# Heartfirey/UCOD-DPL

Measured on AMD Instinct MI355X. Metric: training images/sec at 3x518x518, DINOv2-B (frozen backbone fwd + DBA/APM/discriminator train step), higher is better.
Workload: dtype f16; 1 GPU; BASELINE configs[1]: dinov2_vitb14 @518x518, batch 32/GPU, full APM+DBA+discriminator step, decoder path f32 (1x1 conv as a three-way bf16 split on the matrix pipe: f32-equivalent), backbone fp16 MFMA; global_batch=32, parallelism=dp1, backbone_last_layer=key-minimal (identical key output; 279.6 of 303.1 GFLOP/img), random_init_weights=True, residual_stream=fp16, ln_fold=True

## Files before the change

ucod_dpl_amd/csrc/dba.hip:

```cpp
#include "common.h"
#include "../../include/ucod_dpl.h"

namespace ucod {

constexpr int E = 64;
constexpr float NORM_EPS = 1e-12f;

__global__ __launch_bounds__(256) void colnorm_kernel(const float* __restrict__ d, int ld_c, int c0, const float* __restrict__ emb,
                                                      float* __restrict__ norm, int HW) {
  __shared__ float red[16];
  const int c = blockIdx.x, b = blockIdx.y;
  const float e = emb[c];
  const float* row = d + ((long)b * ld_c + c0 + c) * HW;
  float s = 0.f;
#pragma unroll 8
  for (int p = threadIdx.x; p < HW; p += 256) {
    const float u = row[p] * e;
    s = fmaf(u, u, s);
  }
  s = block_sum(s, red);
  if (threadIdx.x == 0) norm[b * 128 + c] = fmaxf(sqrtf(s), NORM_EPS);
}

__global__ __launch_bounds__(256) void heads_fwd_kernel(const float* __restrict__ d, int ld_c, int c0, const float* __restrict__ emb,
                                                        const float* __restrict__ norm, const float* __restrict__ head_w,
                                                        const float* __restrict__ head_b, float* __restrict__ fg,
                                                        float* __restrict__ bg, float* __restrict__ sdiag, int HW) {
  __shared__ float kf[128], hw[128];
  __shared__ float red[16];
  const int b = blockIdx.y, tid = threadIdx.x;
  if (tid < 128) {
    kf[tid] = emb[tid] / norm[b * 128 + tid];
    hw[tid] = head_w[tid];
  }
  __syncthreads();
  const int p = blockIdx.x * 256 + tid;
  float s2 = 0.f;
  if (p < HW) {
    const float* dp = d + ((long)b * ld_c + c0) * HW + p;
    float accf = head_b[0], accb = head_b[1], s = 0.f;
    for (int c0 = 0; c0 < E; c0 += 16) {
      float v1[16], v2[16];
#pragma unroll
      for (int j = 0; j < 16; ++j) {
        v1[j] = dp[(long)(c0 + j) * HW];
        v2[j] = dp[(long)(c0 + j + E) * HW];
      }
      __builtin_amdgcn_sched_barrier(0);
#pragma unroll
      for (int j = 0; j < 16; ++j) {
        const int c = c0 + j;
        const float d1 = v1[j], d2 = v2[j];
        const float f1 = d1 * kf[c], f2 = d2 * kf[c + E];
        accf = fmaf(hw[c], sigmoid_gate(f1 * d1) + d1, accf);
        accb = fmaf(hw[c + E], sigmoid_gate(f2 * d2) + d2, accb);
        s = fmaf(f1, f2, s);
      }
    }
    fg[(long)b * HW + p] = accf;
    if (bg) bg[(long)b * HW + p] = accb;
    s2 = s * s;
  }
  if (sdiag) {
    s2 = block_sum(s2, red);
    if (tid == 0) atomicAdd(&sdiag[b], s2);
  }
}

constexpr int GCH = 512;
constexpr int GK = 64;
constexpr int GLD = 129;
__global__ __launch_bounds__(256, 2) void gram_partial_kernel(const float* __restrict__ d, int ld_c, int c0,
                                                           const float* __restrict__ emb, const float* __restrict__ norm,
                                                           float* __restrict__ partial, int HW, int S) {
  __shared__ float Fs[2][GK * GLD];
  const int tid = threadIdx.x, lane = tid & 63, wave = tid >> 6;
  const int b = blockIdx.y, ps = blockIdx.x * GCH, pe = min(ps + GCH, HW);
  const float* dbase = d + ((long)b * ld_c + c0) * HW;
  const int sk = tid & 63, srow = tid >> 6;
  const int br = wave >> 1, rt = wave & 1;
  float kf[32];
#pragma unroll
  for (int i = 0; i < 32; ++i) kf[i] = emb[srow + 4 * i] / norm[b * 128 + srow + 4 * i];
  f32x16 acc[2];
#pragma unroll
  for (int i = 0; i < 16; ++i) { acc[0][i] = 0.f; acc[1][i] = 0.f; }

  float r[32];
  auto gload = [&](int k0) {
    const int k = k0 + sk;
    const float* src = dbase + (k < pe ? k : pe - 1);
    const float live = k < pe ? 1.f : 0.f;
#pragma unroll
    for (int i = 0; i < 32; ++i) r[i] = src[(long)(srow + 4 * i) * HW];
#pragma unroll
    for (int i = 0; i < 32; ++i) r[i] *= kf[i] * live;
  };
  auto lstore = [&](int buf) {
#pragma unroll
    for (int i = 0; i < 32; ++i) Fs[buf][sk * GLD + srow + 4 * i] = r[i];
  };
  const int nt = (pe - ps + GK - 1) / GK;
  gload(ps);
  lstore(0);
  for (int t = 0; t < nt; ++t) {
    __syncthreads();
    const bool more = t + 1 < nt;
    if (more) gload(ps + (t + 1) * GK);
    const float* fs = Fs[t & 1];
#pragma unroll 8
    for (int kk = 0; kk < GK; kk += 2) {
      const int k = kk + (lane >> 5);
      const float a = fs[k * GLD + br * 64 + rt * 32 + (lane & 31)];
      const float b0 = fs[k * GLD + br * 64 + (lane & 31)];
      const float b1 = fs[k * GLD + br * 64 + 32 + (lane & 31)];
      acc[0] = __builtin_amdgcn_mfma_f32_32x32x2f32(a, b0, acc[0], 0, 0, 0);
      acc[1] = __builtin_amdgcn_mfma_f32_32x32x2f32(a, b1, acc[1], 0, 0, 0);
    }
    if (more) lstore((t + 1) & 1);
  }
  float* out = partial + (((long)b * S + blockIdx.x) * 2 + br) * (E * E);
#pragma unroll
  for (int ct = 0; ct < 2; ++ct)
#pragma unroll
    for (int rg = 0; rg < 16; ++rg) {
      const int i = rt * 32 + (rg & 3) + 8 * (rg >> 2) + 4 * (lane >> 5);
      const int j = ct * 32 + (lane & 31);
      out[i * E + j] = acc[ct][rg];
    }
}

constexpr int FIN_Y = E * E / 256;
__global__ __launch_bounds__(256) void gram_finalize_kernel(const float* __restrict__ partial, float* __restrict__ gram,
                                                            float* __restrict__ trace, int S) {
  __shared__ float red[16];
  const int b = blockIdx.x, i = blockIdx.y * 256 + threadIdx.x;
  float g1 = 0.f, g2 = 0.f;
  for (int s = 0; s < S; ++s) {
    const float* p = partial + (((long)b * S + s) * 2) * (E * E);
    g1 += p[i];
    g2 += p[E * E + i];
  }
  gram[((long)b * 2 + 0) * (E * E) + i] = g1;
  gram[((long)b * 2 + 1) * (E * E) + i] = g2;
  const float tr = block_sum(g1 * g2, red);
  if (threadIdx.x == 0) trace[b * FIN_Y + blockIdx.y] = tr;
}

__global__ void orth_loss_kernel(const float* __restrict__ trace, const float* __restrict__ sdiag, float* __restrict__ loss, int B,
                                 double inv_z) {
  if (threadIdx.x == 0 && blockIdx.x == 0) {
    double t = 0.0;
    for (int b = 0; b < B; ++b) {
      double tb = 0.0;
      for (int y = 0; y < FIN_Y; ++y) tb += (double)trace[b * FIN_Y + y];
      t += tb - (double)sdiag[b];
    }
    loss[0] = (float)(t * inv_z);
  }
}

__global__ __launch_bounds__(256, 2) void dba_bwd_a_kernel(const float* __restrict__ d, int ld_c, int c0, const float* __restrict__ emb,
                                                           const float* __restrict__ norm, const float* __restrict__ head_w,
                                                           const float* __restrict__ gram, const float* __restrict__ gfg,
                                                           const float* __restrict__ gbg, float coef ,
                                                           float* __restrict__ gfeat, int HW) {
  __shared__ float G[2][E * E];
  __shared__ float kf[128], hw[128];
  const int b = blockIdx.y, tid = threadIdx.x, lane = tid & 63, wave = tid >> 6;
  const int l31 = lane & 31, h5 = lane >> 5;
  for (int i = tid; i < 2 * E * E; i += 256) (&G[0][0])[i] = gram[(long)b * 2 * E * E + i];
  if (tid < 128) {
    kf[tid] = emb[tid] / norm[b * 128 + tid];
    hw[tid] = head_w[tid];
  }
  __syncthreads();
  const int pbase = blockIdx.x * 256 + wave * 64;
  int px[2];
  bool ok[2];
#pragma unroll
  for (int ct = 0; ct < 2; ++ct) {
    const int p = pbase + ct * 32 + l31;
    ok[ct] = p < HW;
    px[ct] = ok[ct] ? p : HW - 1;
  }
  const float* dp = d + ((long)b * ld_c + c0) * HW;

  f32x16 a1[2][2], a2[2][2];
#pragma unroll
  for (int i = 0; i < 16; ++i) {
    a1[0][0][i] = a1[0][1][i] = a1[1][0][i] = a1[1][1][i] = 0.f;
    a2[0][0][i] = a2[0][1][i] = a2[1][0][i] = a2[1][1][i] = 0.f;
  }
  float spart[2] = {0.f, 0.f};
  for (int kk0 = 0; kk0 < E; kk0 += 16) {
    float r1[8][2], r2[8][2];
#pragma unroll
    for (int j = 0; j < 8; ++j) {
      const int k = kk0 + 2 * j + h5;
#pragma unroll
      for (int ct = 0; ct < 2; ++ct) {
        r1[j][ct] = dp[(long)k * HW + px[ct]];
        r2[j][ct] = dp[(long)(k + E) * HW + px[ct]];
      }
    }
    __builtin_amdgcn_sched_barrier(0);
#pragma unroll
    for (int j = 0; j < 8; ++j) {
      const int k = kk0 + 2 * j + h5;
      const float k1 = kf[k], k2 = kf[E + k];
      float f1[2], f2[2];
#pragma unroll
      for (int ct = 0; ct < 2; ++ct) {
        f1[ct] = r1[j][ct] * k1;
        f2[ct] = r2[j][ct] * k2;
        spart[ct] = fmaf(f1[ct], f2[ct], spart[ct]);
      }
#pragma unroll
      for (int rt = 0; rt < 2; ++rt) {
        const float g2 = G[1][k * E + rt * 32 + l31];
        const float g1 = G[0][k * E + rt * 32 + l31];
#pragma unroll
        for (int ct = 0; ct < 2; ++ct) {
          a1[rt][ct] = __builtin_amdgcn_mfma_f32_32x32x2f32(g2, f1[ct], a1[rt][ct], 0, 0, 0);
          a2[rt][ct] = __builtin_amdgcn_mfma_f32_32x32x2f32(g1, f2[ct], a2[rt][ct], 0, 0, 0);
        }
      }
    }
  }
  float* gp = gfeat + (long)b * 128 * HW;
#pragma unroll
  for (int ct = 0; ct < 2; ++ct) {
    const float s = spart[ct] + __shfl_xor(spart[ct], 32, 64);
    const long gi = (long)b * HW + px[ct];
    const float g1 = gfg[gi], g2 = gbg[gi];
#pragma unroll
    for (int rt = 0; rt < 2; ++rt)
#pragma unroll
      for (int r = 0; r < 16; ++r) {
        const int c = rt * 32 + (r & 3) + 8 * (r >> 2) + 4 * h5;
        const float d1 = dp[(long)c * HW + px[ct]], d2 = dp[(long)(c + E) * HW + px[ct]];
        const float f1 = d1 * kf[c], f2 = d2 * kf[c + E];
        const float s1 = sigmoid_gate(f1 * d1), s2 = sigmoid_gate(f2 * d2);
        if (ok[ct]) {
          gp[(long)c * HW + px[ct]] = coef * (a1[rt][ct][r] - s * f2) + g1 * hw[c] * s1 * (1.f - s1) * d1;
          gp[(long)(c + E) * HW + px[ct]] = coef * (a2[rt][ct][r] - s * f1) + g2 * hw[c + E] * s2 * (1.f - s2) * d2;
        }
      }
  }
}

__global__ __launch_bounds__(256) void dba_bwd_b_kernel(const float* __restrict__ d, int ld_c, int c0, const float* __restrict__ emb,
                                                        const float* __restrict__ norm, const float* __restrict__ head_w,
                                                        const float* __restrict__ gfg, const float* __restrict__ gbg,
                                                        const float* __restrict__ gfeat, float* __restrict__ gd,
                                                        float* __restrict__ g_head_w, float* __restrict__ g_head_b,
                                                        float* __restrict__ g_dec_bias, int HW) {
  __shared__ float red[16];
  const int c = blockIdx.x, b = blockIdx.y, tid = threadIdx.x;
  const float e = emb[c], n = norm[b * 128 + c], k = e / n, w = head_w[c];
  const float* drow = d + ((long)b * ld_c + c0 + c) * HW;
  const float* grow = gfeat + ((long)b * 128 + c) * HW;
  const float* gup = (c < E ? gfg : gbg) + (long)b * HW;
  float* orow = gd + ((long)b * 128 + c) * HW;
  float r = 0.f;
#pragma unroll 8
  for (int p = tid; p < HW; p += 256) r = fmaf(drow[p] * k, grow[p], r);
  r = block_sum(r, red);
  const bool clamped = (n <= NORM_EPS);
  float sgd = 0.f, sga = 0.f, sg_up = 0.f;
  for (int p0 = tid; p0 < HW; p0 += 256 * 6) {
    float dv6[6], gf6[6], g6[6];
#pragma unroll
    for (int j = 0; j < 6; ++j) {
      const int p = p0 + 256 * j, pc = p < HW ? p : HW - 1;
      dv6[j] = drow[pc];
      gf6[j] = grow[pc];
      g6[j] = gup[pc];
    }
#pragma unroll
    for (int j = 0; j < 6; ++j) {
      const int p = p0 + 256 * j;
      if (p >= HW) break;
      const float dv = dv6[j], f = dv * k, gf = gf6[j], g = g6[j];
      const float sg = sigmoid_gate(f * dv);
      const float gu = clamped ? gf / NORM_EPS : (gf - f * r) / n;
      const float o = fmaf(gu, e, g * w * fmaf(sg * (1.f - sg), f, 1.f));
      orow[p] = o;
      sgd += o;
      sga = fmaf(g, sg + dv, sga);
      sg_up += g;
    }
  }
  sgd = block_sum(sgd, red);
  sga = block_sum(sga, red);
  if (tid == 0) {
    atomicAdd(&g_dec_bias[c], sgd);
    atomicAdd(&g_head_w[c], sga);
  }
  if (c == 0 || c == E) {
    sg_up = block_sum(sg_up, red);
    if (tid == 0) atomicAdd(&g_head_b[c == E ? 1 : 0], sg_up);
  }
}

}

using namespace ucod;

extern "C" int ucod_dba_colnorm(const float* d, int ld_c, int c0, const float* emb, float* norm, int B, int HW, void* stream) {
  if (!d || !emb || !norm || B <= 0 || HW <= 0 || c0 < 0 || c0 + 128 > ld_c) return UCOD_EINVAL;
  UCOD_PROF(PROF_DBA_COLNORM, stream);
  hipLaunchKernelGGL(colnorm_kernel, dim3(128, B), dim3(256), 0, (hipStream_t)stream, d, ld_c, c0, emb, norm, HW);
  UCOD_CHECK_LAUNCH();
  return UCOD_OK;
}

extern "C" int ucod_dba_heads_fwd(const float* d, int ld_c, int c0, const float* emb, const float* norm, const float* head_w,
                                  const float* head_b, float* fg, float* bg, float* sdiag, int B, int HW, void* stream) {
  if (!d || !emb || !norm || !head_w || !head_b || !fg || B <= 0 || HW <= 0 || c0 < 0 || c0 + 128 > ld_c) return UCOD_EINVAL;
  hipStream_t s = (hipStream_t)stream;
  UCOD_PROF(PROF_DBA_HEADS, s);
  if (sdiag && !ucod::accumulators_prezeroed()) {
    hipError_t e = hipMemsetAsync(sdiag, 0, sizeof(float) * B, s);
    if (e != hipSuccess) return (int)e;
  }
  hipLaunchKernelGGL(heads_fwd_kernel, dim3(cdiv(HW, 256), B), dim3(256), 0, s, d, ld_c, c0, emb, norm, head_w, head_b, fg, bg, sdiag, HW);
  UCOD_CHECK_LAUNCH();
  return UCOD_OK;
}

extern "C" size_t ucod_orth_workspace_bytes(int B, int HW) {
  const size_t S = (size_t)cdiv(HW, GCH);
  return ((size_t)B * S * 2 * E * E + (size_t)B * FIN_Y) * sizeof(float);
}

extern "C" int ucod_orth_gram_fwd(const float* d, int ld_c, int c0, const float* emb, const float* norm, const float* sdiag,
                                  float* gram, float* loss, void* ws, int B, int HW, void* stream) {
  if (!d || !emb || !norm || !sdiag || !gram || !loss || !ws || B <= 0 || HW <= 0 || c0 < 0 || c0 + 128 > ld_c) return UCOD_EINVAL;
  hipStream_t s = (hipStream_t)stream;
  UCOD_PROF(PROF_ORTH, s);
  const int S = cdiv(HW, GCH);
  float* partial = (float*)ws;
  float* trace = partial + (size_t)B * S * 2 * E * E;
  hipLaunchKernelGGL(gram_partial_kernel, dim3(S, B), dim3(256), 0, s, d, ld_c, c0, emb, norm, partial, HW, S);
  hipLaunchKernelGGL(gram_finalize_kernel, dim3(B, FIN_Y), dim3(256), 0, s, partial, gram, trace, S);
  const double inv_z = 1.0 / ((double)B * (double)HW * (double)HW);
  hipLaunchKernelGGL(orth_loss_kernel, dim3(1), dim3(64), 0, s, trace, sdiag, loss, B, inv_z);
  UCOD_CHECK_LAUNCH();
  return UCOD_OK;
}

extern "C" size_t ucod_dba_bwd_workspace_bytes(int B, int HW) { return (size_t)B * 128 * HW * sizeof(float); }

extern "C" int ucod_dba_bwd(const float* d, int ld_c, int c0, const float* emb, const float* norm, const float* head_w,
                            const float* gram, const float* gfg, const float* gbg, float gextra, float* gd, float* g_head_w,
                            float* g_head_b, float* g_dec_bias, void* ws, int B, int HW, void* stream) {
  if (!d || !emb || !norm || !head_w || !gram || !gfg || !gbg || !gd || !g_head_w || !g_head_b || !g_dec_bias || !ws || B <= 0 ||
      HW <= 0 || c0 < 0 || c0 + 128 > ld_c)
    return UCOD_EINVAL;
  hipStream_t s = (hipStream_t)stream;
  float* gfeat = (float*)ws;
  UCOD_PROF(PROF_DBA_BWD, s);
  hipError_t e = hipSuccess;
  if (ucod::accumulators_prezeroed()) {
  } else if (g_head_w == g_dec_bias + 128 && g_head_b == g_head_w + 128) {
    e = hipMemsetAsync(g_dec_bias, 0, sizeof(float) * 258, s);
  } else {
    e = hipMemsetAsync(g_head_w, 0, sizeof(float) * 128, s);
    if (e == hipSuccess) e = hipMemsetAsync(g_head_b, 0, sizeof(float) * 2, s);
    if (e == hipSuccess) e = hipMemsetAsync(g_dec_bias, 0, sizeof(float) * 128, s);
  }
  if (e != hipSuccess) return (int)e;
  const float coef = (float)(2.0 * (double)gextra / ((double)B * (double)HW * (double)HW));
  hipLaunchKernelGGL(dba_bwd_a_kernel, dim3(cdiv(HW, 256), B), dim3(256), 0, s, d, ld_c, c0, emb, norm, head_w, gram, gfg, gbg, coef, gfeat, HW);
  hipLaunchKernelGGL(dba_bwd_b_kernel, dim3(128, B), dim3(256), 0, s, d, ld_c, c0, emb, norm, head_w, gfg, gbg, gfeat, gd, g_head_w, g_head_b, g_dec_bias, HW);
  UCOD_CHECK_LAUNCH();
  return UCOD_OK;
}
```

Measured before the change: 3390 images/s.

## Split DBA gram and backward kernels into smaller tiles for occupancy and pipelining

The gram partial kernel is split across a new grid z dimension, one per 64-channel half. Each wave now owns a single 32x32 accumulator, and LDS operand reads are software-pipelined with register double-buffered global loads. The backward-A kernel handles 32 pixels per wave instead of 64, halving accumulator registers so occupancy can rise to 4 blocks. The backward-B kernel gains a variant that holds all per-row values in registers when HW fits, avoiding a second global read pass. These changes aim to raise occupancy and hide latency, at the cost of more blocks and duplicated loads of the d tensor.

```diff
diff --git a/ucod_dpl_amd/csrc/dba.hip b/ucod_dpl_amd/csrc/dba.hip
--- a/ucod_dpl_amd/csrc/dba.hip
+++ b/ucod_dpl_amd/csrc/dba.hip
@@ -69,65 +69,79 @@
 
 constexpr int GCH = 512;
 constexpr int GK = 64;
-constexpr int GLD = 129;
-__global__ __launch_bounds__(256, 2) void gram_partial_kernel(const float* __restrict__ d, int ld_c, int c0,
+constexpr int GLD = 65;
+constexpr int GRW = E / 4;
+__global__ __launch_bounds__(256, 4) void gram_partial_kernel(const float* __restrict__ d, int ld_c, int c0,
                                                            const float* __restrict__ emb, const float* __restrict__ norm,
                                                            float* __restrict__ partial, int HW, int S) {
   __shared__ float Fs[2][GK * GLD];
-  const int tid = threadIdx.x, lane = tid & 63, wave = tid >> 6;
-  const int b = blockIdx.y, ps = blockIdx.x * GCH, pe = min(ps + GCH, HW);
-  const float* dbase = d + ((long)b * ld_c + c0) * HW;
-  const int sk = tid & 63, srow = tid >> 6;
-  const int br = wave >> 1, rt = wave & 1;
-  float kf[32];
-#pragma unroll
-  for (int i = 0; i < 32; ++i) kf[i] = emb[srow + 4 * i] / norm[b * 128 + srow + 4 * i];
-  f32x16 acc[2];
-#pragma unroll
-  for (int i = 0; i < 16; ++i) { acc[0][i] = 0.f; acc[1][i] = 0.f; }
-
-  float r[32];
-  auto gload = [&](int k0) {
+  const int tid = threadIdx.x, lane = tid & 63, wave = __builtin_amdgcn_readfirstlane(tid >> 6);
+  const int b = blockIdx.y, br = blockIdx.z, ps = blockIdx.x * GCH, pe = min(ps + GCH, HW);
+  const float* dbase = d + ((long)b * ld_c + c0 + br * E) * HW;
+  const int sk = lane, srow = wave;
+  const int rt = wave >> 1, ct = wave & 1;
+  float kf[GRW];
+#pragma unroll
+  for (int i = 0; i < GRW; ++i) kf[i] = emb[br * E + srow + 4 * i] / norm[b * 128 + br * E + srow + 4 * i];
+  f32x16 acc;
+#pragma unroll
+  for (int i = 0; i < 16; ++i) acc[i] = 0.f;
+
+  float r0[GRW], r1[GRW];
+  auto gload = [&](float (&r)[GRW], int k0) {
     const int k = k0 + sk;
-    const float* src = dbase + (k < pe ? k : pe - 1);
-    const float live = k < pe ? 1.f : 0.f;
-#pragma unroll
-    for (int i = 0; i < 32; ++i) r[i] = src[(long)(srow + 4 * i) * HW];
-#pragma unroll
-    for (int i = 0; i < 32; ++i) r[i] *= kf[i] * live;
+    const unsigned ko = k < pe ? k : pe - 1;
+#pragma unroll
+    for (int i = 0; i < GRW; ++i) r[i] = (dbase + (long)(srow + 4 * i) * HW)[ko];
   };
-  auto lstore = [&](int buf) {
-#pragma unroll
-    for (int i = 0; i < 32; ++i) Fs[buf][sk * GLD + srow + 4 * i] = r[i];
+  auto lstore = [&](const float (&r)[GRW], int k0, int buf) {
+    const float live = k0 + sk < pe ? 1.f : 0.f;
+#pragma unroll
+    for (int i = 0; i < GRW; ++i) Fs[buf][sk * GLD + srow + 4 * i] = r[i] * (kf[i] * live);
+  };
+  auto tile = [&](int buf) {
+    const float* fs = Fs[buf] + (lane >> 5) * GLD + (lane & 31);
+    float av[2][4], bv[2][4];
+    auto oread = [&](int g, float (&a)[4], float (&bb)[4]) {
+#pragma unroll
+      for (int j = 0; j < 4; ++j) {
+        a[j] = fs[(8 * g + 2 * j) * GLD + rt * 32];
+        bb[j] = fs[(8 * g + 2 * j) * GLD + ct * 32];
+      }
+    };
+    oread(0, av[0], bv[0]);
+#pragma unroll
+    for (int g = 0; g < GK / 8; ++g) {
+      if (g + 1 < GK / 8) oread(g + 1, av[(g + 1) & 1], bv[(g + 1) & 1]);
+      __builtin_amdgcn_sched_barrier(0);
+#pragma unroll
+      for (int j = 0; j < 4; ++j) acc = __builtin_amdgcn_mfma_f32_32x32x2f32(av[g & 1][j], bv[g & 1][j], acc, 0, 0, 0);
+    }
   };
   const int nt = (pe - ps + GK - 1) / GK;
-  gload(ps);
-  lstore(0);
-  for (int t = 0; t < nt; ++t) {
+  gload(r0, ps);
+  gload(r1, ps + GK);
+  lstore(r0, ps, 0);
+  for (int t = 0; t < nt; t += 2) {
     __syncthreads();
-    const bool more = t + 1 < nt;
-    if (more) gload(ps + (t + 1) * GK);
-    const float* fs = Fs[t & 1];
-#pragma unroll 8
-    for (int kk = 0; kk < GK; kk += 2) {
-      const int k = kk + (lane >> 5);
-      const float a = fs[k * GLD + br * 64 + rt * 32 + (lane & 31)];
-      const float b0 = fs[k * GLD + br * 64 + (lane & 31)];
-      const float b1 = fs[k * GLD + br * 64 + 32 + (lane & 31)];
-      acc[0] = __builtin_amdgcn_mfma_f32_32x32x2f32(a, b0, acc[0], 0, 0, 0);
-      acc[1] = __builtin_amdgcn_mfma_f32_32x32x2f32(a, b1, acc[1], 0, 0, 0);
-    }
-    if (more) lstore((t + 1) & 1);
+    gload(r0, ps + (t + 2) * GK);
+    __builtin_amdgcn_sched_barrier(0);
+    tile(0);
+    lstore(r1, ps + (t + 1) * GK, 1);
+    if (t + 1 >= nt) break;
+    __syncthreads();
+    gload(r1, ps + (t + 3) * GK);
+    __builtin_amdgcn_sched_barrier(0);
+    tile(1);
+    lstore(r0, ps + (t + 2) * GK, 0);
   }
   float* out = partial + (((long)b * S + blockIdx.x) * 2 + br) * (E * E);
 #pragma unroll
-  for (int ct = 0; ct < 2; ++ct)
-#pragma unroll
-    for (int rg = 0; rg < 16; ++rg) {
-      const int i = rt * 32 + (rg & 3) + 8 * (rg >> 2) + 4 * (lane >> 5);
-      const int j = ct * 32 + (lane & 31);
-      out[i * E + j] = acc[ct][rg];
-    }
+  for (int rg = 0; rg < 16; ++rg) {
+    const int i = rt * 32 + (rg & 3) + 8 * (rg >> 2) + 4 * (lane >> 5);
+    const int j = ct * 32 + (lane & 31);
+    out[i * E + j] = acc[rg];
+  }
 }
 
 constexpr int FIN_Y = E * E / 256;
@@ -160,7 +174,7 @@
   }
 }
 
-__global__ __launch_bounds__(256, 2) void dba_bwd_a_kernel(const float* __restrict__ d, int ld_c, int c0, const float* __restrict__ emb,
+__global__ __launch_bounds__(256, 4) void dba_bwd_a_kernel(const float* __restrict__ d, int ld_c, int c0, const float* __restrict__ emb,
                                                            const float* __restrict__ norm, const float* __restrict__ head_w,
                                                            const float* __restrict__ gram, const float* __restrict__ gfg,
                                                            const float* __restrict__ gbg, float coef ,
@@ -175,82 +189,85 @@
     hw[tid] = head_w[tid];
   }
   __syncthreads();
-  const int pbase = blockIdx.x * 256 + wave * 64;
-  int px[2];
-  bool ok[2];
-#pragma unroll
-  for (int ct = 0; ct < 2; ++ct) {
-    const int p = pbase + ct * 32 + l31;
-    ok[ct] = p < HW;
-    px[ct] = ok[ct] ? p : HW - 1;
-  }
+  const int p = (blockIdx.x * 4 + wave) * 32 + l31;
+  const bool ok = p < HW;
+  const int px = ok ? p : HW - 1;
   const float* dp = d + ((long)b * ld_c + c0) * HW;
-
-  f32x16 a1[2][2], a2[2][2];
-#pragma unroll
-  for (int i = 0; i < 16; ++i) {
-    a1[0][0][i] = a1[0][1][i] = a1[1][0][i] = a1[1][1][i] = 0.f;
-    a2[0][0][i] = a2[0][1][i] = a2[1][0][i] = a2[1][1][i] = 0.f;
-  }
-  float spart[2] = {0.f, 0.f};
-  for (int kk0 = 0; kk0 < E; kk0 += 16) {
-    float r1[8][2], r2[8][2];
-#pragma unroll
-    for (int j = 0; j < 8; ++j) {
+  const unsigned lo1 = (unsigned)(h5 * HW + px);
+  const unsigned lo4 = (unsigned)(4 * h5 * HW + px);
+
+  f32x16 a1[2], a2[2];
+#pragma unroll
+  for (int rt = 0; rt < 2; ++rt)
+#pragma unroll
+    for (int i = 0; i < 16; ++i) a1[rt][i] = a2[rt][i] = 0.f;
+  float spart = 0.f;
+  constexpr int KP = 8;
+  for (int kk0 = 0; kk0 < E; kk0 += 2 * KP) {
+    float r1[KP], r2[KP];
+#pragma unroll
+    for (int j = 0; j < KP; ++j) {
+      const float* row1 = dp + (long)(kk0 + 2 * j) * HW;
+      r1[j] = row1[lo1];
+      r2[j] = (row1 + (long)E * HW)[lo1];
+    }
+    __builtin_amdgcn_sched_barrier(0);
+    float gq[2][2][2], kq[2][2];
+    auto oread = [&](int j, float (&g)[2][2], float (&kk)[2]) {
       const int k = kk0 + 2 * j + h5;
-#pragma unroll
-      for (int ct = 0; ct < 2; ++ct) {
-        r1[j][ct] = dp[(long)k * HW + px[ct]];
-        r2[j][ct] = dp[(long)(k + E) * HW + px[ct]];
-      }
+      kk[0] = kf[k];
+      kk[1] = kf[E + k];
+#pragma unroll
+      for (int rt = 0; rt < 2; ++rt) {
+        g[0][rt] = G[0][k * E + rt * 32 + l31];
+        g[1][rt] = G[1][k * E + rt * 32 + l31];
+      }
+    };
+    oread(0, gq[0], kq[0]);
+#pragma unroll
+    for (int j = 0; j < KP; ++j) {
+      if (j + 1 < KP) oread(j + 1, gq[(j + 1) & 1], kq[(j + 1) & 1]);
+      __builtin_amdgcn_sched_barrier(0);
+      const float f1 = r1[j] * kq[j & 1][0], f2 = r2[j] * kq[j & 1][1];
+      spart = fmaf(f1, f2, spart);
+#pragma unroll
+      for (int rt = 0; rt < 2; ++rt) {
+        a1[rt] = __builtin_amdgcn_mfma_f32_32x32x2f32(gq[j & 1][1][rt], f1, a1[rt], 0, 0, 0);
+        a2[rt] = __builtin_amdgcn_mfma_f32_32x32x2f32(gq[j & 1][0][rt], f2, a2[rt], 0, 0, 0);
+      }
+    }
+  }
+  float* gp = gfeat + (long)b * 128 * HW;
+  const float s = spart + __shfl_xor(spart, 32, 64);
+  const float g1 = gfg[(long)b * HW + px], g2 = gbg[(long)b * HW + px];
+#pragma unroll
+  for (int rt = 0; rt < 2; ++rt) {
+    float dv1[16], dv2[16];
+#pragma unroll
+    for (int r = 0; r < 16; ++r) {
+      const float* drow1 = dp + (long)(rt * 32 + (r & 3) + 8 * (r >> 2)) * HW;
+      dv1[r] = drow1[lo4];
+      dv2[r] = (drow1 + (long)E * HW)[lo4];
     }
     __builtin_amdgcn_sched_barrier(0);
 #pragma unroll
-    for (int j = 0; j < 8; ++j) {
-      const int k = kk0 + 2 * j + h5;
-      const float k1 = kf[k], k2 = kf[E + k];
-      float f1[2], f2[2];
-#pragma unroll
-      for (int ct = 0; ct < 2; ++ct) {
-        f1[ct] = r1[j][ct] * k1;
-        f2[ct] = r2[j][ct] * k2;
-        spart[ct] = fmaf(f1[ct], f2[ct], spart[ct]);
-      }
-#pragma unroll
-      for (int rt = 0; rt < 2; ++rt) {
-        const float g2 = G[1][k * E + rt * 32 + l31];
-        const float g1 = G[0][k * E + rt * 32 + l31];
-#pragma unroll
-        for (int ct = 0; ct < 2; ++ct) {
-          a1[rt][ct] = __builtin_amdgcn_mfma_f32_32x32x2f32(g2, f1[ct], a1[rt][ct], 0, 0, 0);
-          a2[rt][ct] = __builtin_amdgcn_mfma_f32_32x32x2f32(g1, f2[ct], a2[rt][ct], 0, 0, 0);
-        }
-      }
-    }
-  }
-  float* gp = gfeat + (long)b * 128 * HW;
-#pragma unroll
-  for (int ct = 0; ct < 2; ++ct) {
-    const float s = spart[ct] + __shfl_xor(spart[ct], 32, 64);
-    const long gi = (long)b * HW + px[ct];
-    const float g1 = gfg[gi], g2 = gbg[gi];
-#pragma unroll
-    for (int rt = 0; rt < 2; ++rt)
-#pragma unroll
-      for (int r = 0; r < 16; ++r) {
-        const int c = rt * 32 + (r & 3) + 8 * (r >> 2) + 4 * h5;
-        const float d1 = dp[(long)c * HW + px[ct]], d2 = dp[(long)(c + E) * HW + px[ct]];
-        const float f1 = d1 * kf[c], f2 = d2 * kf[c + E];
-        const float s1 = sigmoid_gate(f1 * d1), s2 = sigmoid_gate(f2 * d2);
-        if (ok[ct]) {
-          gp[(long)c * HW + px[ct]] = coef * (a1[rt][ct][r] - s * f2) + g1 * hw[c] * s1 * (1.f - s1) * d1;
-          gp[(long)(c + E) * HW + px[ct]] = coef * (a2[rt][ct][r] - s * f1) + g2 * hw[c + E] * s2 * (1.f - s2) * d2;
-        }
-      }
-  }
-}
-
-__global__ __launch_bounds__(256) void dba_bwd_b_kernel(const float* __restrict__ d, int ld_c, int c0, const float* __restrict__ emb,
+    for (int r = 0; r < 16; ++r) {
+      const int cu = rt * 32 + (r & 3) + 8 * (r >> 2), c = cu + 4 * h5;
+      float* grow1 = gp + (long)cu * HW;
+      const float d1 = dv1[r], d2 = dv2[r];
+      const float f1 = d1 * kf[c], f2 = d2 * kf[c + E];
+      const float s1 = sigmoid_gate(f1 * d1), s2 = sigmoid_gate(f2 * d2);
+      if (ok) {
+        grow1[lo4] = coef * (a1[rt][r] - s * f2) + g1 * hw[c] * s1 * (1.f - s1) * d1;
+        (grow1 + (long)E * HW)[lo4] = coef * (a2[rt][r] - s * f1) + g2 * hw[c + E] * s2 * (1.f - s2) * d2;
+      }
+    }
+  }
+}
+
+constexpr int BPT = 20;
+template <bool HELD>
+__global__ __launch_bounds__(256, 4) void dba_bwd_b_kernel(const float* __restrict__ d, int ld_c, int c0, const float* __restrict__ emb,
                                                         const float* __restrict__ norm, const float* __restrict__ head_w,
                                                         const float* __restrict__ gfg, const float* __restrict__ gbg,
                                                         const float* __restrict__ gfeat, float* __restrict__ gd,
@@ -263,33 +280,57 @@
   const float* grow = gfeat + ((long)b * 128 + c) * HW;
   const float* gup = (c < E ? gfg : gbg) + (long)b * HW;
   float* orow = gd + ((long)b * 128 + c) * HW;
-  float r = 0.f;
+  const bool clamped = (n <= NORM_EPS);
+  float r = 0.f, sgd = 0.f, sga = 0.f, sg_up = 0.f;
+  auto apply = [&](int p, float dv, float gf, float g) {
+    const float f = dv * k;
+    const float sg = sigmoid_gate(f * dv);
+    const float gu = clamped ? gf / NORM_EPS : (gf - f * r) / n;
+    const float o = fmaf(gu, e, g * w * fmaf(sg * (1.f - sg), f, 1.f));
+    orow[p] = o;
+    sgd += o;
+    sga = fmaf(g, sg + dv, sga);
+    sg_up += g;
+  };
+  if constexpr (HELD) {
+    float dvh[BPT], gfh[BPT], gh[BPT];
+#pragma unroll
+    for (int j = 0; j < BPT; ++j) {
+      const unsigned p = tid + 256 * j, pc = p < (unsigned)HW ? p : HW - 1;
+      dvh[j] = drow[pc];
+      gfh[j] = grow[pc];
+    }
+#pragma unroll
+    for (int j = 0; j < BPT; ++j) {
+      const unsigned p = tid + 256 * j, pc = p < (unsigned)HW ? p : HW - 1;
+      gh[j] = gup[pc];
+    }
+#pragma unroll
+    for (int j = 0; j < BPT; ++j)
+      if (tid + 256 * j < HW) r = fmaf(dvh[j] * k, gfh[j], r);
+    r = block_sum(r, red);
+#pragma unroll
+    for (int j = 0; j < BPT; ++j)
+      if (tid + 256 * j < HW) apply(tid + 256 * j, dvh[j], gfh[j], gh[j]);
+  } else {
 #pragma unroll 8
-  for (int p = tid; p < HW; p += 256) r = fmaf(drow[p] * k, grow[p], r);
-  r = block_sum(r, red);
-  const bool clamped = (n <= NORM_EPS);
-  float sgd = 0.f, sga = 0.f, sg_up = 0.f;
-  for (int p0 = tid; p0 < HW; p0 += 256 * 6) {
-    float dv6[6], gf6[6], g6[6];
-#pragma unroll
-    for (int j = 0; j < 6; ++j) {
-      const int p = p0 + 256 * j, pc = p < HW ? p : HW - 1;
-      dv6[j] = drow[pc];
-      gf6[j] = grow[pc];
-      g6[j] = gup[pc];
-    }
-#pragma unroll
-    for (int j = 0; j < 6; ++j) {
-      const int p = p0 + 256 * j;
-      if (p >= HW) break;
-      const float dv = dv6[j], f = dv * k, gf = gf6[j], g = g6[j];
-      const float sg = sigmoid_gate(f * dv);
-      const float gu = clamped ? gf / NORM_EPS : (gf - f * r) / n;
-      const float o = fmaf(gu, e, g * w * fmaf(sg * (1.f - sg), f, 1.f));
-      orow[p] = o;
-      sgd += o;
-      sga = fmaf(g, sg + dv, sga);
-      sg_up += g;
+    for (int p = tid; p < HW; p += 256) r = fmaf(drow[p] * k, grow[p], r);
+    r = block_sum(r, red);
+    for (int p0 = tid; p0 < HW; p0 += 256 * 6) {
+      float dv6[6], gf6[6], g6[6];
+#pragma unroll
+      for (int j = 0; j < 6; ++j) {
+        const int p = p0 + 256 * j, pc = p < HW ? p : HW - 1;
+        dv6[j] = drow[pc];
+        gf6[j] = grow[pc];
+        g6[j] = gup[pc];
+      }
+#pragma unroll
+      for (int j = 0; j < 6; ++j) {
+        const int p = p0 + 256 * j;
+        if (p >= HW) break;
+        apply(p, dv6[j], gf6[j], g6[j]);
+      }
     }
   }
   sgd = block_sum(sgd, red);
@@ -343,7 +384,7 @@
   const int S = cdiv(HW, GCH);
   float* partial = (float*)ws;
   float* trace = partial + (size_t)B * S * 2 * E * E;
-  hipLaunchKernelGGL(gram_partial_kernel, dim3(S, B), dim3(256), 0, s, d, ld_c, c0, emb, norm, partial, HW, S);
+  hipLaunchKernelGGL(gram_partial_kernel, dim3(S, B, 2), dim3(256), 0, s, d, ld_c, c0, emb, norm, partial, HW, S);
   hipLaunchKernelGGL(gram_finalize_kernel, dim3(B, FIN_Y), dim3(256), 0, s, partial, gram, trace, S);
   const double inv_z = 1.0 / ((double)B * (double)HW * (double)HW);
   hipLaunchKernelGGL(orth_loss_kernel, dim3(1), dim3(64), 0, s, trace, sdiag, loss, B, inv_z);
@@ -357,7 +398,7 @@
                             const float* gram, const float* gfg, const float* gbg, float gextra, float* gd, float* g_head_w,
                             float* g_head_b, float* g_dec_bias, void* ws, int B, int HW, void* stream) {
   if (!d || !emb || !norm || !head_w || !gram || !gfg || !gbg || !gd || !g_head_w || !g_head_b || !g_dec_bias || !ws || B <= 0 ||
-      HW <= 0 || c0 < 0 || c0 + 128 > ld_c)
+      HW <= 0 || HW >= (1 << 27)  || c0 < 0 || c0 + 128 > ld_c)
     return UCOD_EINVAL;
   hipStream_t s = (hipStream_t)stream;
   float* gfeat = (float*)ws;
@@ -373,8 +414,11 @@
   }
   if (e != hipSuccess) return (int)e;
   const float coef = (float)(2.0 * (double)gextra / ((double)B * (double)HW * (double)HW));
-  hipLaunchKernelGGL(dba_bwd_a_kernel, dim3(cdiv(HW, 256), B), dim3(256), 0, s, d, ld_c, c0, emb, norm, head_w, gram, gfg, gbg, coef, gfeat, HW);
-  hipLaunchKernelGGL(dba_bwd_b_kernel, dim3(128, B), dim3(256), 0, s, d, ld_c, c0, emb, norm, head_w, gfg, gbg, gfeat, gd, g_head_w, g_head_b, g_dec_bias, HW);
+  hipLaunchKernelGGL(dba_bwd_a_kernel, dim3(cdiv(HW, 128), B), dim3(256), 0, s, d, ld_c, c0, emb, norm, head_w, gram, gfg, gbg, coef, gfeat, HW);
+  if (HW <= 256 * BPT)
+    hipLaunchKernelGGL(dba_bwd_b_kernel<true>, dim3(128, B), dim3(256), 0, s, d, ld_c, c0, emb, norm, head_w, gfg, gbg, gfeat, gd, g_head_w, g_head_b, g_dec_bias, HW);
+  else
+    hipLaunchKernelGGL(dba_bwd_b_kernel<false>, dim3(128, B), dim3(256), 0, s, d, ld_c, c0, emb, norm, head_w, gfg, gbg, gfeat, gd, g_head_w, g_head_b, g_dec_bias, HW);
   UCOD_CHECK_LAUNCH();
   return UCOD_OK;
 }
```

Result: no change. 3389 images/s (-0.0%).
